# r9y9/deepvoice3_pytorch

Measured on NVIDIA H100. Metric: mel-frames/sec training step (B=16,T_mel=800), higher is better.
Workload: dtype f32 via split 16-bit pairs (fp16 pairs forward, bf16 pairs for gradients; 3 wgmma passes per product, fp32 accumulate)

## Files before the change

deepvoice3_pytorch_b200/csrc/tc_common.cuh:

```cuda
#pragma once
#include <cuda.h>
#include <cuda_bf16.h>
#include "common.cuh"

namespace dv3 {
namespace tc {

__device__ __forceinline__ uint32_t smem_u32(const void* p) { return (uint32_t)__cvta_generic_to_shared(p); }

__device__ __forceinline__ void mbar_init(uint64_t* bar, uint32_t count) {
    asm volatile("mbarrier.init.shared::cta.b64 [%0], %1;" ::"r"(smem_u32(bar)), "r"(count));
}
__device__ __forceinline__ void fence_barrier_init() {
    asm volatile("fence.mbarrier_init.release.cluster;" ::: "memory");
}
__device__ __forceinline__ void fence_proxy_async() {
    asm volatile("fence.proxy.async.shared::cta;" ::: "memory");
}
__device__ __forceinline__ void mbar_arrive_expect_tx(uint64_t* bar, uint32_t bytes) {
    asm volatile("mbarrier.arrive.expect_tx.shared::cta.b64 _, [%0], %1;" ::"r"(smem_u32(bar)), "r"(bytes)
                 : "memory");
}
__device__ __forceinline__ void mbar_arrive(uint64_t* bar) {
    asm volatile("mbarrier.arrive.shared::cta.b64 _, [%0];" ::"r"(smem_u32(bar)) : "memory");
}
__device__ __forceinline__ void mbar_wait(uint64_t* bar, uint32_t parity) {
    asm volatile(
        "{\n"
        ".reg .pred p;\n"
        "DV3_WAIT:\n"
        "mbarrier.try_wait.parity.shared::cta.b64 p, [%0], %1;\n"
        "@p bra DV3_DONE;\n"
        "bra DV3_WAIT;\n"
        "DV3_DONE:\n"
        "}\n" ::"r"(smem_u32(bar)),
        "r"(parity)
        : "memory");
}

__device__ __forceinline__ void tma_load_3d(void* smem_dst, const CUtensorMap* map, uint64_t* bar, int c0, int c1,
                                            int c2) {
    asm volatile(
        "cp.async.bulk.tensor.3d.shared::cluster.global.mbarrier::complete_tx::bytes [%0], [%1, {%3, %4, %5}], [%2];"
        ::"r"(smem_u32(smem_dst)), "l"(map), "r"(smem_u32(bar)), "r"(c0), "r"(c1), "r"(c2)
        : "memory");
}
__device__ __forceinline__ void prefetch_tmap(const CUtensorMap* map) {
    asm volatile("prefetch.tensormap [%0];" ::"l"(map) : "memory");
}
__device__ __forceinline__ void tma_store_3d(const CUtensorMap* map, const void* smem_src, int c0, int c1, int c2) {
    asm volatile("cp.async.bulk.tensor.3d.global.shared::cta.bulk_group [%0, {%2, %3, %4}], [%1];"
                 ::"l"(map), "r"(smem_u32(smem_src)), "r"(c0), "r"(c1), "r"(c2)
                 : "memory");
}
__device__ __forceinline__ void bulk_commit() { asm volatile("cp.async.bulk.commit_group;" ::: "memory"); }
__device__ __forceinline__ void bulk_wait_read() { asm volatile("cp.async.bulk.wait_group.read 0;" ::: "memory"); }
__device__ __forceinline__ void bulk_wait() { asm volatile("cp.async.bulk.wait_group 0;" ::: "memory"); }
__device__ __forceinline__ void mbar_arrive_cnt(uint64_t* bar, uint32_t count) {
    asm volatile("mbarrier.arrive.shared::cta.b64 _, [%0], %1;" ::"r"(smem_u32(bar)), "r"(count) : "memory");
}
__device__ __forceinline__ void named_bar_sync(int id, int threads) {
    asm volatile("bar.sync %0, %1;" ::"r"(id), "r"(threads) : "memory");
}

template <int N>
__device__ __forceinline__ void setmaxnreg_dec() { asm volatile("setmaxnreg.dec.sync.aligned.u32 %0;" ::"n"(N)); }
template <int N>
__device__ __forceinline__ void setmaxnreg_inc() { asm volatile("setmaxnreg.inc.sync.aligned.u32 %0;" ::"n"(N)); }

__device__ __forceinline__ void wgmma_fence() { asm volatile("wgmma.fence.sync.aligned;" ::: "memory"); }
__device__ __forceinline__ void wgmma_commit() { asm volatile("wgmma.commit_group.sync.aligned;" ::: "memory"); }
template <int N>
__device__ __forceinline__ void wgmma_wait() { asm volatile("wgmma.wait_group.sync.aligned %0;" ::"n"(N) : "memory"); }
__device__ __forceinline__ int frag_row(int i, int warp_in_wg, int lane) {
    return 16 * warp_in_wg + (lane >> 2) + 8 * ((i >> 1) & 1);
}
__device__ __forceinline__ int frag_col(int i, int lane) { return 8 * (i >> 2) + 2 * (lane & 3) + (i & 1); }

__device__ __forceinline__ uint64_t make_wgmma_desc(uint32_t saddr, uint32_t lbo, uint32_t sbo, uint32_t layout) {
    uint64_t d = 0;
    d |= (uint64_t)((saddr & 0x3FFFF) >> 4);
    d |= (uint64_t)((lbo >> 4) & 0x3FFF) << 16;
    d |= (uint64_t)((sbo >> 4) & 0x3FFF) << 32;
    d |= (uint64_t)layout << 62;
    return d;
}
constexpr uint32_t WG_SW128 = 1, WG_SW64 = 2;

template <int TA, int TB>
__device__ __forceinline__ void wgmma_f16_n64(float* d, uint64_t a, uint64_t b, uint32_t acc) {
    asm volatile(
        "{\n.reg .pred p;\nsetp.ne.b32 p, %34, 0;\n"
        "wgmma.mma_async.sync.aligned.m64n64k16.f32.f16.f16 {%0, %1, %2, %3, %4, %5, %6, %7, %8, %9, %10, %11, %12, %13, %14, %15, %16, %17, %18, %19, %20, %21, %22, %23, %24, %25, %26, %27, %28, %29, %30, %31}, %32, %33, p, 1, 1, %35, %36;\n}\n"
        : "+f"(d[0]), "+f"(d[1]), "+f"(d[2]), "+f"(d[3]), "+f"(d[4]), "+f"(d[5]), "+f"(d[6]), "+f"(d[7]), "+f"(d[8]), "+f"(d[9]), "+f"(d[10]), "+f"(d[11]), "+f"(d[12]), "+f"(d[13]), "+f"(d[14]), "+f"(d[15]), "+f"(d[16]), "+f"(d[17]), "+f"(d[18]), "+f"(d[19]), "+f"(d[20]), "+f"(d[21]), "+f"(d[22]), "+f"(d[23]), "+f"(d[24]), "+f"(d[25]), "+f"(d[26]), "+f"(d[27]), "+f"(d[28]), "+f"(d[29]), "+f"(d[30]), "+f"(d[31])
        : "l"(a), "l"(b), "r"(acc), "n"(TA), "n"(TB));
}
template <int TA, int TB>
__device__ __forceinline__ void wgmma_bf16_n64(float* d, uint64_t a, uint64_t b, uint32_t acc) {
    asm volatile(
        "{\n.reg .pred p;\nsetp.ne.b32 p, %34, 0;\n"
        "wgmma.mma_async.sync.aligned.m64n64k16.f32.bf16.bf16 {%0, %1, %2, %3, %4, %5, %6, %7, %8, %9, %10, %11, %12, %13, %14, %15, %16, %17, %18, %19, %20, %21, %22, %23, %24, %25, %26, %27, %28, %29, %30, %31}, %32, %33, p, 1, 1, %35, %36;\n}\n"
        : "+f"(d[0]), "+f"(d[1]), "+f"(d[2]), "+f"(d[3]), "+f"(d[4]), "+f"(d[5]), "+f"(d[6]), "+f"(d[7]), "+f"(d[8]), "+f"(d[9]), "+f"(d[10]), "+f"(d[11]), "+f"(d[12]), "+f"(d[13]), "+f"(d[14]), "+f"(d[15]), "+f"(d[16]), "+f"(d[17]), "+f"(d[18]), "+f"(d[19]), "+f"(d[20]), "+f"(d[21]), "+f"(d[22]), "+f"(d[23]), "+f"(d[24]), "+f"(d[25]), "+f"(d[26]), "+f"(d[27]), "+f"(d[28]), "+f"(d[29]), "+f"(d[30]), "+f"(d[31])
        : "l"(a), "l"(b), "r"(acc), "n"(TA), "n"(TB));
}
template <int TA, int TB>
__device__ __forceinline__ void wgmma_f16_n128(float* d, uint64_t a, uint64_t b, uint32_t acc) {
    asm volatile(
        "{\n.reg .pred p;\nsetp.ne.b32 p, %66, 0;\n"
        "wgmma.mma_async.sync.aligned.m64n128k16.f32.f16.f16 {%0, %1, %2, %3, %4, %5, %6, %7, %8, %9, %10, %11, %12, %13, %14, %15, %16, %17, %18, %19, %20, %21, %22, %23, %24, %25, %26, %27, %28, %29, %30, %31, %32, %33, %34, %35, %36, %37, %38, %39, %40, %41, %42, %43, %44, %45, %46, %47, %48, %49, %50, %51, %52, %53, %54, %55, %56, %57, %58, %59, %60, %61, %62, %63}, %64, %65, p, 1, 1, %67, %68;\n}\n"
        : "+f"(d[0]), "+f"(d[1]), "+f"(d[2]), "+f"(d[3]), "+f"(d[4]), "+f"(d[5]), "+f"(d[6]), "+f"(d[7]), "+f"(d[8]), "+f"(d[9]), "+f"(d[10]), "+f"(d[11]), "+f"(d[12]), "+f"(d[13]), "+f"(d[14]), "+f"(d[15]), "+f"(d[16]), "+f"(d[17]), "+f"(d[18]), "+f"(d[19]), "+f"(d[20]), "+f"(d[21]), "+f"(d[22]), "+f"(d[23]), "+f"(d[24]), "+f"(d[25]), "+f"(d[26]), "+f"(d[27]), "+f"(d[28]), "+f"(d[29]), "+f"(d[30]), "+f"(d[31]), "+f"(d[32]), "+f"(d[33]), "+f"(d[34]), "+f"(d[35]), "+f"(d[36]), "+f"(d[37]), "+f"(d[38]), "+f"(d[39]), "+f"(d[40]), "+f"(d[41]), "+f"(d[42]), "+f"(d[43]), "+f"(d[44]), "+f"(d[45]), "+f"(d[46]), "+f"(d[47]), "+f"(d[48]), "+f"(d[49]), "+f"(d[50]), "+f"(d[51]), "+f"(d[52]), "+f"(d[53]), "+f"(d[54]), "+f"(d[55]), "+f"(d[56]), "+f"(d[57]), "+f"(d[58]), "+f"(d[59]), "+f"(d[60]), "+f"(d[61]), "+f"(d[62]), "+f"(d[63])
        : "l"(a), "l"(b), "r"(acc), "n"(TA), "n"(TB));
}
template <int TA, int TB>
__device__ __forceinline__ void wgmma_bf16_n128(float* d, uint64_t a, uint64_t b, uint32_t acc) {
    asm volatile(
        "{\n.reg .pred p;\nsetp.ne.b32 p, %66, 0;\n"
        "wgmma.mma_async.sync.aligned.m64n128k16.f32.bf16.bf16 {%0, %1, %2, %3, %4, %5, %6, %7, %8, %9, %10, %11, %12, %13, %14, %15, %16, %17, %18, %19, %20, %21, %22, %23, %24, %25, %26, %27, %28, %29, %30, %31, %32, %33, %34, %35, %36, %37, %38, %39, %40, %41, %42, %43, %44, %45, %46, %47, %48, %49, %50, %51, %52, %53, %54, %55, %56, %57, %58, %59, %60, %61, %62, %63}, %64, %65, p, 1, 1, %67, %68;\n}\n"
        : "+f"(d[0]), "+f"(d[1]), "+f"(d[2]), "+f"(d[3]), "+f"(d[4]), "+f"(d[5]), "+f"(d[6]), "+f"(d[7]), "+f"(d[8]), "+f"(d[9]), "+f"(d[10]), "+f"(d[11]), "+f"(d[12]), "+f"(d[13]), "+f"(d[14]), "+f"(d[15]), "+f"(d[16]), "+f"(d[17]), "+f"(d[18]), "+f"(d[19]), "+f"(d[20]), "+f"(d[21]), "+f"(d[22]), "+f"(d[23]), "+f"(d[24]), "+f"(d[25]), "+f"(d[26]), "+f"(d[27]), "+f"(d[28]), "+f"(d[29]), "+f"(d[30]), "+f"(d[31]), "+f"(d[32]), "+f"(d[33]), "+f"(d[34]), "+f"(d[35]), "+f"(d[36]), "+f"(d[37]), "+f"(d[38]), "+f"(d[39]), "+f"(d[40]), "+f"(d[41]), "+f"(d[42]), "+f"(d[43]), "+f"(d[44]), "+f"(d[45]), "+f"(d[46]), "+f"(d[47]), "+f"(d[48]), "+f"(d[49]), "+f"(d[50]), "+f"(d[51]), "+f"(d[52]), "+f"(d[53]), "+f"(d[54]), "+f"(d[55]), "+f"(d[56]), "+f"(d[57]), "+f"(d[58]), "+f"(d[59]), "+f"(d[60]), "+f"(d[61]), "+f"(d[62]), "+f"(d[63])
        : "l"(a), "l"(b), "r"(acc), "n"(TA), "n"(TB));
}
template <int TA, int TB>
__device__ __forceinline__ void wgmma_f16_n256(float* d, uint64_t a, uint64_t b, uint32_t acc) {
    asm volatile(
        "{\n.reg .pred p;\nsetp.ne.b32 p, %130, 0;\n"
        "wgmma.mma_async.sync.aligned.m64n256k16.f32.f16.f16 {%0, %1, %2, %3, %4, %5, %6, %7, %8, %9, %10, %11, %12, %13, %14, %15, %16, %17, %18, %19, %20, %21, %22, %23, %24, %25, %26, %27, %28, %29, %30, %31, %32, %33, %34, %35, %36, %37, %38, %39, %40, %41, %42, %43, %44, %45, %46, %47, %48, %49, %50, %51, %52, %53, %54, %55, %56, %57, %58, %59, %60, %61, %62, %63, %64, %65, %66, %67, %68, %69, %70, %71, %72, %73, %74, %75, %76, %77, %78, %79, %80, %81, %82, %83, %84, %85, %86, %87, %88, %89, %90, %91, %92, %93, %94, %95, %96, %97, %98, %99, %100, %101, %102, %103, %104, %105, %106, %107, %108, %109, %110, %111, %112, %113, %114, %115, %116, %117, %118, %119, %120, %121, %122, %123, %124, %125, %126, %127}, %128, %129, p, 1, 1, %131, %132;\n}\n"
        : "+f"(d[0]), "+f"(d[1]), "+f"(d[2]), "+f"(d[3]), "+f"(d[4]), "+f"(d[5]), "+f"(d[6]), "+f"(d[7]), "+f"(d[8]), "+f"(d[9]), "+f"(d[10]), "+f"(d[11]), "+f"(d[12]), "+f"(d[13]), "+f"(d[14]), "+f"(d[15]), "+f"(d[16]), "+f"(d[17]), "+f"(d[18]), "+f"(d[19]), "+f"(d[20]), "+f"(d[21]), "+f"(d[22]), "+f"(d[23]), "+f"(d[24]), "+f"(d[25]), "+f"(d[26]), "+f"(d[27]), "+f"(d[28]), "+f"(d[29]), "+f"(d[30]), "+f"(d[31]), "+f"(d[32]), "+f"(d[33]), "+f"(d[34]), "+f"(d[35]), "+f"(d[36]), "+f"(d[37]), "+f"(d[38]), "+f"(d[39]), "+f"(d[40]), "+f"(d[41]), "+f"(d[42]), "+f"(d[43]), "+f"(d[44]), "+f"(d[45]), "+f"(d[46]), "+f"(d[47]), "+f"(d[48]), "+f"(d[49]), "+f"(d[50]), "+f"(d[51]), "+f"(d[52]), "+f"(d[53]), "+f"(d[54]), "+f"(d[55]), "+f"(d[56]), "+f"(d[57]), "+f"(d[58]), "+f"(d[59]), "+f"(d[60]), "+f"(d[61]), "+f"(d[62]), "+f"(d[63]), "+f"(d[64]), "+f"(d[65]), "+f"(d[66]), "+f"(d[67]), "+f"(d[68]), "+f"(d[69]), "+f"(d[70]), "+f"(d[71]), "+f"(d[72]), "+f"(d[73]), "+f"(d[74]), "+f"(d[75]), "+f"(d[76]), "+f"(d[77]), "+f"(d[78]), "+f"(d[79]), "+f"(d[80]), "+f"(d[81]), "+f"(d[82]), "+f"(d[83]), "+f"(d[84]), "+f"(d[85]), "+f"(d[86]), "+f"(d[87]), "+f"(d[88]), "+f"(d[89]), "+f"(d[90]), "+f"(d[91]), "+f"(d[92]), "+f"(d[93]), "+f"(d[94]), "+f"(d[95]), "+f"(d[96]), "+f"(d[97]), "+f"(d[98]), "+f"(d[99]), "+f"(d[100]), "+f"(d[101]), "+f"(d[102]), "+f"(d[103]), "+f"(d[104]), "+f"(d[105]), "+f"(d[106]), "+f"(d[107]), "+f"(d[108]), "+f"(d[109]), "+f"(d[110]), "+f"(d[111]), "+f"(d[112]), "+f"(d[113]), "+f"(d[114]), "+f"(d[115]), "+f"(d[116]), "+f"(d[117]), "+f"(d[118]), "+f"(d[119]), "+f"(d[120]), "+f"(d[121]), "+f"(d[122]), "+f"(d[123]), "+f"(d[124]), "+f"(d[125]), "+f"(d[126]), "+f"(d[127])
        : "l"(a), "l"(b), "r"(acc), "n"(TA), "n"(TB));
}
template <int TA, int TB>
__device__ __forceinline__ void wgmma_bf16_n256(float* d, uint64_t a, uint64_t b, uint32_t acc) {
    asm volatile(
        "{\n.reg .pred p;\nsetp.ne.b32 p, %130, 0;\n"
        "wgmma.mma_async.sync.aligned.m64n256k16.f32.bf16.bf16 {%0, %1, %2, %3, %4, %5, %6, %7, %8, %9, %10, %11, %12, %13, %14, %15, %16, %17, %18, %19, %20, %21, %22, %23, %24, %25, %26, %27, %28, %29, %30, %31, %32, %33, %34, %35, %36, %37, %38, %39, %40, %41, %42, %43, %44, %45, %46, %47, %48, %49, %50, %51, %52, %53, %54, %55, %56, %57, %58, %59, %60, %61, %62, %63, %64, %65, %66, %67, %68, %69, %70, %71, %72, %73, %74, %75, %76, %77, %78, %79, %80, %81, %82, %83, %84, %85, %86, %87, %88, %89, %90, %91, %92, %93, %94, %95, %96, %97, %98, %99, %100, %101, %102, %103, %104, %105, %106, %107, %108, %109, %110, %111, %112, %113, %114, %115, %116, %117, %118, %119, %120, %121, %122, %123, %124, %125, %126, %127}, %128, %129, p, 1, 1, %131, %132;\n}\n"
        : "+f"(d[0]), "+f"(d[1]), "+f"(d[2]), "+f"(d[3]), "+f"(d[4]), "+f"(d[5]), "+f"(d[6]), "+f"(d[7]), "+f"(d[8]), "+f"(d[9]), "+f"(d[10]), "+f"(d[11]), "+f"(d[12]), "+f"(d[13]), "+f"(d[14]), "+f"(d[15]), "+f"(d[16]), "+f"(d[17]), "+f"(d[18]), "+f"(d[19]), "+f"(d[20]), "+f"(d[21]), "+f"(d[22]), "+f"(d[23]), "+f"(d[24]), "+f"(d[25]), "+f"(d[26]), "+f"(d[27]), "+f"(d[28]), "+f"(d[29]), "+f"(d[30]), "+f"(d[31]), "+f"(d[32]), "+f"(d[33]), "+f"(d[34]), "+f"(d[35]), "+f"(d[36]), "+f"(d[37]), "+f"(d[38]), "+f"(d[39]), "+f"(d[40]), "+f"(d[41]), "+f"(d[42]), "+f"(d[43]), "+f"(d[44]), "+f"(d[45]), "+f"(d[46]), "+f"(d[47]), "+f"(d[48]), "+f"(d[49]), "+f"(d[50]), "+f"(d[51]), "+f"(d[52]), "+f"(d[53]), "+f"(d[54]), "+f"(d[55]), "+f"(d[56]), "+f"(d[57]), "+f"(d[58]), "+f"(d[59]), "+f"(d[60]), "+f"(d[61]), "+f"(d[62]), "+f"(d[63]), "+f"(d[64]), "+f"(d[65]), "+f"(d[66]), "+f"(d[67]), "+f"(d[68]), "+f"(d[69]), "+f"(d[70]), "+f"(d[71]), "+f"(d[72]), "+f"(d[73]), "+f"(d[74]), "+f"(d[75]), "+f"(d[76]), "+f"(d[77]), "+f"(d[78]), "+f"(d[79]), "+f"(d[80]), "+f"(d[81]), "+f"(d[82]), "+f"(d[83]), "+f"(d[84]), "+f"(d[85]), "+f"(d[86]), "+f"(d[87]), "+f"(d[88]), "+f"(d[89]), "+f"(d[90]), "+f"(d[91]), "+f"(d[92]), "+f"(d[93]), "+f"(d[94]), "+f"(d[95]), "+f"(d[96]), "+f"(d[97]), "+f"(d[98]), "+f"(d[99]), "+f"(d[100]), "+f"(d[101]), "+f"(d[102]), "+f"(d[103]), "+f"(d[104]), "+f"(d[105]), "+f"(d[106]), "+f"(d[107]), "+f"(d[108]), "+f"(d[109]), "+f"(d[110]), "+f"(d[111]), "+f"(d[112]), "+f"(d[113]), "+f"(d[114]), "+f"(d[115]), "+f"(d[116]), "+f"(d[117]), "+f"(d[118]), "+f"(d[119]), "+f"(d[120]), "+f"(d[121]), "+f"(d[122]), "+f"(d[123]), "+f"(d[124]), "+f"(d[125]), "+f"(d[126]), "+f"(d[127])
        : "l"(a), "l"(b), "r"(acc), "n"(TA), "n"(TB));
}

template <int N, int TA, int TB>
__device__ __forceinline__ void wgmma_mma(bool bf16, float* d, uint64_t a, uint64_t b, uint32_t acc) {
    if (N == 64) { if (bf16) wgmma_bf16_n64<TA, TB>(d, a, b, acc); else wgmma_f16_n64<TA, TB>(d, a, b, acc); }
    if (N == 128) { if (bf16) wgmma_bf16_n128<TA, TB>(d, a, b, acc); else wgmma_f16_n128<TA, TB>(d, a, b, acc); }
    if (N == 256) { if (bf16) wgmma_bf16_n256<TA, TB>(d, a, b, acc); else wgmma_f16_n256<TA, TB>(d, a, b, acc); }
}

}

int encode_tmap_bf16_3d(CUtensorMap* map, const void* base, uint64_t d0, uint64_t d1, uint64_t d2,
                        uint64_t stride1_bytes, uint64_t stride2_bytes, uint32_t box0, uint32_t box1);

}
```

deepvoice3_pytorch_b200/csrc/tc_gemm.cu:

```cuda
#include "tc_common.cuh"
#include "tc_ring.cuh"
#include "../../include/dv3b200.h"

namespace dv3 {

using namespace tc;

constexpr int TC_CONV_THREADS = 512;
constexpr int TC_PRODUCER_REGS = 24;
constexpr int TC_CONSUMER_REGS = 168;
constexpr int TC_EPILOGUE_REGS = 152;
static_assert(TC_PRODUCER_REGS <= 65536 / TC_CONV_THREADS && TC_CONSUMER_REGS >= 65536 / TC_CONV_THREADS &&
              TC_EPILOGUE_REGS >= 65536 / TC_CONV_THREADS, "setmaxnreg direction of each warpgroup");
static_assert(128 * TC_PRODUCER_REGS + 256 * TC_CONSUMER_REGS + 128 * TC_EPILOGUE_REGS <= 65536, "register file");
constexpr int MAX_TAPS_TC = 8;
enum { TC_GATED = 0, TC_CONV = 1 };

struct TcMaps { CUtensorMap a[2]; CUtensorMap b[2]; };

struct TcParams {
    int T;
    int Nc;
    int rows_per_tap;
    int k, kb_n;
    int tap_off[MAX_TAPS_TC];
    const float* bias; const float* spk; const float* res;
    float* y; float* save_a; float* save_s;
    int gate_mode, residual;
    float* out; const float* e1; const float* e2; float alpha; int addmode, relu;
    float p_drop; const unsigned long long* seed_ptr; uint32_t salt;
    float gmain;
    int operand_bf16;
    int tma_out;
};

template <int BK> struct SwizzleOf;
template <> struct SwizzleOf<64> { static constexpr uint32_t layout = WG_SW128, sbo = 1024; };
template <> struct SwizzleOf<32> { static constexpr uint32_t layout = WG_SW64, sbo = 512; };

template <int BK>
__device__ __forceinline__ uint64_t make_desc(uint32_t saddr) {
    return make_wgmma_desc(saddr, 16, SwizzleOf<BK>::sbo, SwizzleOf<BK>::layout);
}


template <int NC>
__device__ __forceinline__ int dense_at(int c) {
    const int r = threadIdx.x & 127;
    return (r >> 5) * NC * 32 + c * 32 + ((((r >> 2) & 7) ^ (c & 7)) << 2) + (r & 3);
}

struct TcOutMaps { CUtensorMap out[3]; CUtensorMap res; };

struct Handoff { float* tile; float* staging; uint64_t* acc_empty; uint64_t* in_full; };

__device__ __forceinline__ void release_tile(const Handoff& h, bool tma) {
    if (!tma) mbar_arrive(h.acc_empty);
    else if ((threadIdx.x & 127) == 0) {
        bulk_commit();
        bulk_wait_read();
        mbar_arrive_cnt(h.acc_empty, 128);
    }
}

template <int BR>
__device__ __forceinline__ void stage_residual(const TcParams& p, const TcOutMaps& om, const Handoff& h, int a_row0,
                                               int a_z, int b_row0) {
    if (!p.tma_out || !((p.gate_mode != 0) || p.residual) || (threadIdx.x & 127) != 0) return;
    mbar_arrive_expect_tx(h.in_full, 128 * BR * 4);
#pragma unroll
    for (int q = 0; q < 4; ++q) tma_load_3d(h.staging + q * BR * 32, &om.res, h.in_full, a_row0 + 32 * q, b_row0, a_z);
}

template <int BR>
__device__ __forceinline__ void epilogue_gated(const TcParams& p, const TcOutMaps& om, const Handoff& h, int n,
                                               int a_row0, int a_z, int b_row0) {
    constexpr int NC = 2 * BR;
    const int t = a_row0 + (threadIdx.x & 127), b = a_z, C = p.Nc;
    const bool tv = t < p.T, tma = p.tma_out != 0;
    const float* __restrict__ bias = p.bias;
    const float* __restrict__ res = p.res;
    const float* __restrict__ spk = p.spk;
    float* __restrict__ yo = p.y;
    float* __restrict__ ao = p.save_a;
    float* __restrict__ so = p.save_s;
    float* tile = h.tile;
    float* st = h.staging;
    const bool need_res = (p.gate_mode != 0) || p.residual;
    const size_t base = ((size_t)b * C + b_row0) * p.T + (tv ? t : 0);
    if (need_res) {
        if (tma) mbar_wait(h.in_full, n & 1);
        else {
#pragma unroll 8
            for (int c = 0; c < BR; ++c) st[dense_at<BR>(c)] = tv ? __ldg(&res[base + (size_t)c * p.T]) : 0.f;
        }
    }
#pragma unroll 1
    for (int c32 = 0; c32 < BR; c32 += 32) {
        float sp[32], ba[32], bb[32];
        const size_t cb = base + (size_t)c32 * p.T;
#pragma unroll
        for (int i = 0; i < 32; ++i) {
            ba[i] = __ldg(&bias[b_row0 + c32 + i]);
            bb[i] = __ldg(&bias[C + b_row0 + c32 + i]);
            if (spk) sp[i] = tv ? __ldg(&spk[cb + (size_t)i * p.T]) : 0.f;
        }
#pragma unroll
        for (int i = 0; i < 32; ++i) {
            const int cl = c32 + i;
            float va = tile[dense_at<NC>(cl)];
            if (spk) va += sp[i];
            const float a = va + ba[i];
            const float s = sigmoidf_(tile[dense_at<NC>(BR + cl)] + bb[i]);
            const float rr = need_res ? st[dense_at<BR>(cl)] : 0.f;
            float y;
            if (p.gate_mode == 0) {
                y = a * s;
                if (p.residual) y = (y + rr) * 0.70710678118654752f;
            } else {
                y = s * a + (1.f - s) * rr;
            }
            st[dense_at<BR>(cl)] = y;
            tile[dense_at<NC>(cl)] = a;
            tile[dense_at<NC>(BR + cl)] = s;
        }
    }
    if (tma) {
        fence_proxy_async();
        named_bar_sync(1, 128);
        if ((threadIdx.x & 127) == 0) {
#pragma unroll
            for (int q = 0; q < 4; ++q) {
                const int t0 = a_row0 + 32 * q;
                if (t0 >= p.T) break;
                tma_store_3d(&om.out[0], st + q * BR * 32, t0, b_row0, b);
                if (ao) tma_store_3d(&om.out[1], tile + q * NC * 32, t0, b_row0, b);
                if (so) tma_store_3d(&om.out[2], tile + q * NC * 32 + BR * 32, t0, b_row0, b);
            }
        }
    } else if (tv) {
#pragma unroll 8
        for (int c = 0; c < BR; ++c) {
            const size_t idx = base + (size_t)c * p.T;
            yo[idx] = st[dense_at<BR>(c)];
            if (ao) ao[idx] = tile[dense_at<NC>(c)];
            if (so) so[idx] = tile[dense_at<NC>(BR + c)];
        }
    }
    release_tile(h, tma);
}

template <int NCOLS>
__device__ __forceinline__ void epilogue_conv(const TcParams& p, const TcOutMaps& om, const Handoff& h, int a_row0,
                                              int a_z, int b_row0) {
    const int t = a_row0 + (threadIdx.x & 127), b = a_z;
    const bool tv = t < p.T, tma = p.tma_out != 0;
    const DropCfg drop = make_drop(p.p_drop, p.seed_ptr, p.salt);
    const float* __restrict__ bias = p.bias;
    const float* __restrict__ e1 = p.e1;
    const float* __restrict__ e2 = p.e2;
    float* __restrict__ out = p.out;
    float* tile = h.tile;
    const size_t base = ((size_t)b * p.Nc + b_row0) * p.T + (tv ? t : 0);
#pragma unroll 1
    for (int c32 = 0; c32 < NCOLS; c32 += 32) {
        float bz[32], v[32], x2[32];
        const int n0 = b_row0 + c32;
        const size_t cb = base + (size_t)c32 * p.T;
#pragma unroll
        for (int i = 0; i < 32; ++i) {
            const bool ok = tv && n0 + i < p.Nc;
            bz[i] = (bias && n0 + i < p.Nc) ? __ldg(&bias[n0 + i]) : 0.f;
            v[i] = (p.addmode != 0 && ok) ? __ldg(&e1[cb + (size_t)i * p.T]) : 0.f;
            x2[i] = (p.addmode == 2 && ok) ? __ldg(&e2[cb + (size_t)i * p.T]) : 0.f;
        }
#pragma unroll
        for (int i = 0; i < 32; ++i) {
            float& d = tile[dense_at<NCOLS>(c32 + i)];
            float g = d * drop_scale(drop, (uint32_t)(cb + (size_t)i * p.T));
            if (bias) g += bz[i];
            if (p.addmode == 1) g += p.alpha * v[i];
            else if (p.addmode == 2) g += v[i] * (1.f - x2[i]);
            if (p.relu) g = fmaxf(g, 0.f);
            d = g;
        }
    }
    if (tma) {
        fence_proxy_async();
        named_bar_sync(1, 128);
        if ((threadIdx.x & 127) == 0) {
#pragma unroll
            for (int q = 0; q < 4; ++q) {
                const int t0 = a_row0 + 32 * q;
                if (t0 >= p.T) break;
                tma_store_3d(&om.out[0], tile + q * NCOLS * 32, t0, b_row0, b);
            }
        }
    } else if (tv) {
#pragma unroll 8
        for (int c = 0; c < NCOLS; ++c)
            if (b_row0 + c < p.Nc) out[base + (size_t)c * p.T] = tile[dense_at<NCOLS>(c)];
    }
    release_tile(h, tma);
}

template <class Cfg, int NPL, class Decode, class Load, class Mma, class Gmain, class Epilogue, class Stage>
__device__ __forceinline__ void tc_pipeline(const TcMaps& maps, int num_units, Decode decode, Load load, Mma mma,
                                            Gmain gmain, Epilogue epilogue, Stage stage) {
    static_assert(NPL == 1 || NPL == 2, "one or two operand planes");
    static_assert(Cfg::NCOLS <= 128, "main + cross accumulators must fit in the registers of a consumer thread");
    static_assert(Cfg::STAGES >= 2, "pipeline needs at least two stages");
    constexpr int STAGE = Cfg::STAGE, STAGES = Cfg::STAGES;
    constexpr int NR = Cfg::NCOLS / 2;
    pdl_trigger();
    extern __shared__ uint8_t smem_raw[];
    uint8_t* smem = smem_raw + ((1024 - (smem_u32(smem_raw) & 1023)) & 1023);
    float* acc_tile = reinterpret_cast<float*>(smem + STAGES * STAGE);
    uint64_t* full = reinterpret_cast<uint64_t*>(smem + STAGES * STAGE + Cfg::ACC_TILE + Cfg::STAGING);
    uint64_t* empty = full + STAGES;
    uint64_t* acc_full = empty + STAGES;
    uint64_t* acc_empty = acc_full + 1;
    uint64_t* in_full = acc_empty + 1;
    const int warp = threadIdx.x >> 5, lane = threadIdx.x & 31;

    if (threadIdx.x == 0) {
#pragma unroll
        for (int pl = 0; pl < NPL; ++pl) prefetch_tmap(&maps.a[pl]);
#pragma unroll
        for (int pl = 0; pl < NPL; ++pl) prefetch_tmap(&maps.b[pl]);
        for (int s = 0; s < STAGES; ++s) { mbar_init(&full[s], 1); mbar_init(&empty[s], 2); }
        mbar_init(acc_full, 256);
        mbar_init(acc_empty, 128);
        mbar_init(in_full, 1);
        fence_barrier_init();
    }
    __syncthreads();
    pdl_wait();

    if (warp >= 12) {
        setmaxnreg_inc<TC_EPILOGUE_REGS>();
        const Handoff h = {acc_tile, acc_tile + Cfg::ACC_TILE / 4, acc_empty, in_full};
        if (blockIdx.x < num_units) stage(decode(blockIdx.x), h);
        int n = 0;
        for (int u = blockIdx.x; u < num_units; u += gridDim.x, ++n) {
            const auto w = decode(u);
            mbar_wait(acc_full, n & 1);
            epilogue(w, n, h);
            if (u + gridDim.x < num_units) stage(decode(u + gridDim.x), h);
        }
        if ((threadIdx.x & 127) == 0) bulk_wait();
    } else if (warp >= 8) {
        setmaxnreg_dec<TC_PRODUCER_REGS>();
        if (warp == 8 && lane == 0) {
            int it = 0;
            for (int u = blockIdx.x; u < num_units; u += gridDim.x) {
                const auto w = decode(u);
                for (int kit = 0; kit < w.n_iters; ++kit, ++it) {
                    const int s = it % STAGES, ph = (it / STAGES) & 1;
                    mbar_wait(&empty[s], ph ^ 1);
                    mbar_arrive_expect_tx(&full[s], STAGE);
                    load(w, kit, smem + s * STAGE, &full[s]);
                }
            }
        }
    } else {
        setmaxnreg_inc<TC_CONSUMER_REGS>();
        const int wg = warp >> 2, wq = warp & 3;
        float acc[NR], xacc[NPL == 2 ? NR : 1];
        int it = 0, n = 0;
        for (int u = blockIdx.x; u < num_units; u += gridDim.x, ++n) {
            const auto w = decode(u);
#pragma unroll
            for (int i = 0; i < NR; ++i) {
                acc[i] = 0.f;
                if constexpr (NPL == 2) xacc[i] = 0.f;
            }
            for (int kit = 0; kit < w.n_iters; ++kit, ++it) {
                const int s = it % STAGES, ph = (it / STAGES) & 1;
                mbar_wait(&full[s], ph);
                wgmma_fence();
                mma(smem + s * STAGE, wg, acc, xacc);
                wgmma_commit();
                wgmma_wait<1>();
                if (kit > 0 && (threadIdx.x & 127) == 0) mbar_arrive(&empty[(it - 1) % STAGES]);
            }
            wgmma_wait<0>();
            if (w.n_iters > 0 && (threadIdx.x & 127) == 0) mbar_arrive(&empty[(it - 1) % STAGES]);
            const float gm = gmain(w);
            mbar_wait(acc_empty, (n & 1) ^ 1);
            const int sw = (((wq & 1) << 2) | (lane >> 4)) ^ ((lane & 3) << 1);
            float* const frag0 = Cfg::DENSE ? acc_tile + (2 * wg + (wq >> 1)) * Cfg::NCOLS * 32 + (lane & 3) * 64 +
                                                  ((lane >> 2) & 3)
                                            : acc_tile;
#pragma unroll
            for (int i = 0; i < NR; ++i) {
                float* dst = Cfg::DENSE
                    ? frag0 + (i >> 2) * 256 + (i & 1) * 32 + ((sw ^ (i & 3)) << 2)
                    : &acc_tile[(64 * wg + frag_row(i, wq, lane)) * Cfg::ACC_PITCH + frag_col(i, lane)];
                if constexpr (NPL == 2) *dst = fmaf(xacc[i], LO_INV, acc[i] * gm);
                else *dst = acc[i] * gm;
            }
            mbar_arrive(acc_full);
        }
    }
}

template <int MODE, int NBOX, int BR, int BK, bool BF16, int NPL>
__global__ void __launch_bounds__(TC_CONV_THREADS, 1)
tc_conv_kernel(const __grid_constant__ TcMaps maps, const __grid_constant__ TcOutMaps om,
               const __grid_constant__ TcParams p, int tiles_x, int tiles_y, int num_tiles) {
    using Cfg = TcCfg<NBOX, BK, BR, NPL>;
    constexpr int NCOLS = Cfg::NCOLS;
    constexpr int TILE = 128 * BK * 2, TILE_B = BR * BK * 2;
    constexpr int B_OFF = NPL * TILE;
    constexpr int A_HALF = 64 * BK * 2;
    const int n_iters = p.k * p.kb_n;

    struct Tile { int a_row0, a_z, b_row0, b_row1, n_iters; };
    auto decode = [&](int tile) {
        Tile w;
        const int ty = tile % tiles_y, r = tile / tiles_y;
        w.a_z = r / tiles_x;
        w.a_row0 = (r % tiles_x) * 128;
        if (MODE == TC_GATED) { w.b_row0 = ty * BR; w.b_row1 = p.Nc + ty * BR; }
        else { w.b_row0 = ty * BR * NBOX; w.b_row1 = w.b_row0 + BR; }
        w.n_iters = n_iters;
        return w;
    };
    auto load = [&](const Tile& w, int kit, uint8_t* st, uint64_t* bar) {
        const int j = kit / p.kb_n, kb = kit - j * p.kb_n;
        const int ax = kb * BK, ay = w.a_row0 + p.tap_off[j];
        const int by0 = j * p.rows_per_tap + w.b_row0, by1 = j * p.rows_per_tap + w.b_row1;
#pragma unroll
        for (int pl = 0; pl < NPL; ++pl) {
            tma_load_3d(st + pl * TILE, &maps.a[pl], bar, ax, ay, w.a_z);
            uint8_t* bdst = st + B_OFF + pl * NBOX * TILE_B;
            tma_load_3d(bdst, &maps.b[pl], bar, ax, by0, 0);
            if (NBOX == 2) tma_load_3d(bdst + TILE_B, &maps.b[pl], bar, ax, by1, 0);
        }
    };
    auto mma = [&](const uint8_t* st, int wg, float* acc, float* xacc) {
        const uint32_t sa = smem_u32(st) + wg * A_HALF, sb = smem_u32(st + B_OFF);
#pragma unroll
        for (int kk = 0; kk < BK / 16; ++kk) {
            const uint32_t ko = kk * 32;
            const uint64_t a0 = make_desc<BK>(sa + ko), b0 = make_desc<BK>(sb + ko);
            wgmma_mma<NCOLS, 0, 0>(BF16, acc, a0, b0, 1);
            if constexpr (NPL == 2) {
                const uint64_t a1 = make_desc<BK>(sa + TILE + ko), b1 = make_desc<BK>(sb + NBOX * TILE_B + ko);
                wgmma_mma<NCOLS, 0, 0>(BF16, xacc, a0, b1, 1);
                wgmma_mma<NCOLS, 0, 0>(BF16, xacc, a1, b0, 1);
            }
        }
    };
    auto gmain = [&](const Tile&) { return p.gmain; };
    auto epilogue = [&](const Tile& w, int n, const Handoff& h) {
        if (MODE == TC_GATED) epilogue_gated<BR>(p, om, h, n, w.a_row0, w.a_z, w.b_row0);
        else epilogue_conv<NCOLS>(p, om, h, w.a_row0, w.a_z, w.b_row0);
    };
    auto stage = [&](const Tile& w, const Handoff& h) {
        if (MODE == TC_GATED) stage_residual<BR>(p, om, h, w.a_row0, w.a_z, w.b_row0);
    };
    tc_pipeline<Cfg, NPL>(maps, num_tiles, decode, load, mma, gmain, epilogue, stage);
}

struct TcMnParams {
    int T, B, Mw, Nw, k;
    int tap_off[MAX_TAPS_TC];
    int nsplit, batches_per_split, kb_n;
    int tiles_n, tiles_m, num_units;
    float* dw; long long split_stride;
    int msplit; long long s_m, s_mh, s_n, s_j;
    float gcoef;
};

template <int NPL>
__global__ void __launch_bounds__(TC_CONV_THREADS, 1)
tc_wgrad_mn_kernel(const __grid_constant__ TcMaps maps, const __grid_constant__ TcMnParams p) {
    using Cfg = WgCfg<NPL>;
    constexpr int A_PL = 2 * WG_BOX, B_PL = 2 * WG_BOX;
    constexpr uint32_t LBO = 4096, SBO = 1024;

    struct Unit { int m0, n0, j, s, b_beg, n_iters; };
    auto decode = [&](int u) {
        Unit w;
        w.n0 = (u % p.tiles_n) * 128;
        int r = u / p.tiles_n;
        w.m0 = (r % p.tiles_m) * 128;
        r /= p.tiles_m;
        w.j = r % p.k;
        w.s = r / p.k;
        w.b_beg = w.s * p.batches_per_split;
        const int b_end = min(p.B, w.b_beg + p.batches_per_split);
        w.n_iters = (b_end > w.b_beg ? b_end - w.b_beg : 0) * p.kb_n;
        return w;
    };
    auto load = [&](const Unit& w, int kit, uint8_t* st, uint64_t* bar) {
        const int bi = kit / p.kb_n, tc_ = kit - bi * p.kb_n;
        const int b = w.b_beg + bi, t0 = tc_ * 32;
#pragma unroll
        for (int pl = 0; pl < NPL; ++pl) {
#pragma unroll
            for (int h = 0; h < 2; ++h)
                tma_load_3d(st + pl * A_PL + h * WG_BOX, &maps.a[pl], bar, w.m0 + h * 64, t0, b);
#pragma unroll
            for (int q = 0; q < 2; ++q)
                tma_load_3d(st + NPL * A_PL + pl * B_PL + q * WG_BOX, &maps.b[pl], bar, w.n0 + q * 64,
                            t0 + p.tap_off[w.j], b);
        }
    };
    auto mma = [&](const uint8_t* st, int wg, float* acc, float* xacc) {
        const uint32_t sa = smem_u32(st);
#pragma unroll
        for (int kk = 0; kk < 2; ++kk) {
            const uint32_t ko = kk * 16 * 128;
            const uint64_t a0 = make_wgmma_desc(sa + wg * WG_BOX + ko, LBO, SBO, WG_SW128);
            const uint64_t b0 = make_wgmma_desc(sa + NPL * A_PL + ko, LBO, SBO, WG_SW128);
            wgmma_mma<128, 1, 1>(true, acc, a0, b0, 1);
            if constexpr (NPL == 2) {
                const uint64_t a1 = make_wgmma_desc(sa + A_PL + wg * WG_BOX + ko, LBO, SBO, WG_SW128);
                const uint64_t b1 = make_wgmma_desc(sa + 2 * A_PL + B_PL + ko, LBO, SBO, WG_SW128);
                wgmma_mma<128, 1, 1>(true, xacc, a0, b1, 1);
                wgmma_mma<128, 1, 1>(true, xacc, a1, b0, 1);
            }
        }
    };
    auto gmain = [&](const Unit& w) { return 1.f + p.gcoef * (float)(2 * w.n_iters); };
    auto epilogue = [&](const Unit& w, int, const Handoff& h) {
        const float* acc_tile = h.tile;
        const int r = threadIdx.x & 127;
        float* __restrict__ out = p.dw + (size_t)w.s * p.split_stride + (size_t)w.j * p.s_j;
        const int rows = min(128, p.Mw - w.m0), cols = min(128, p.Nw - w.n0);
        if (p.s_n == 1) {
            if (r < cols) {
                float* __restrict__ o = out + w.n0 + r;
#pragma unroll 4
                for (int i = 0; i < rows; ++i) {
                    const int m = w.m0 + i;
                    o[(size_t)(m % p.msplit) * p.s_m + (size_t)(m / p.msplit) * p.s_mh] = acc_tile[i * Cfg::ACC_PITCH + r];
                }
            }
        } else if (r < rows) {
            const int m = w.m0 + r;
            float* __restrict__ o = out + (size_t)(m % p.msplit) * p.s_m + (size_t)(m / p.msplit) * p.s_mh +
                                    (size_t)w.n0 * p.s_n;
            const float* arow = acc_tile + r * Cfg::ACC_PITCH;
#pragma unroll 4
            for (int c = 0; c < cols; ++c) o[(size_t)c * p.s_n] = arow[c];
        }
        mbar_arrive(h.acc_empty);
    };
    tc_pipeline<Cfg, NPL>(maps, p.num_units, decode, load, mma, gmain, epilogue, [](const Unit&, const Handoff&) {});
}

typedef CUresult (*EncodeTiledFn)(CUtensorMap*, CUtensorMapDataType, cuuint32_t, void*, const cuuint64_t*,
                                  const cuuint64_t*, const cuuint32_t*, const cuuint32_t*, CUtensorMapInterleave,
                                  CUtensorMapSwizzle, CUtensorMapL2promotion, CUtensorMapFloatOOBfill);

static EncodeTiledFn encode_fn() {
    static const EncodeTiledFn fn = [] {
        void* f = nullptr;
        cudaDriverEntryPointQueryResult qres;
        cudaError_t e = cudaGetDriverEntryPoint("cuTensorMapEncodeTiled", &f, cudaEnableDefault, &qres);
        return (e == cudaSuccess) ? (EncodeTiledFn)f : (EncodeTiledFn) nullptr;
    }();
    return fn;
}

int encode_tmap_bf16_3d(CUtensorMap* map, const void* base, uint64_t d0, uint64_t d1, uint64_t d2,
                        uint64_t stride1_bytes, uint64_t stride2_bytes, uint32_t box0, uint32_t box1) {
    const EncodeTiledFn enc = encode_fn();
    if (!enc) { set_error("cuTensorMapEncodeTiled entry point unavailable"); return 1; }
    cuuint64_t dims[3] = {d0, d1, d2};
    cuuint64_t strides[2] = {stride1_bytes, stride2_bytes};
    cuuint32_t box[3] = {box0, box1, 1};
    cuuint32_t estr[3] = {1, 1, 1};
    const CUtensorMapSwizzle sw = box0 * 2 == 128 ? CU_TENSOR_MAP_SWIZZLE_128B : CU_TENSOR_MAP_SWIZZLE_64B;
    CUresult r = enc(map, CU_TENSOR_MAP_DATA_TYPE_BFLOAT16, 3, const_cast<void*>(base), dims, strides, box, estr,
                     CU_TENSOR_MAP_INTERLEAVE_NONE, sw, CU_TENSOR_MAP_L2_PROMOTION_L2_256B,
                     CU_TENSOR_MAP_FLOAT_OOB_FILL_NONE);
    if (r != CUDA_SUCCESS) {
        set_error("cuTensorMapEncodeTiled failed (%d): dims=(%llu,%llu,%llu) strides=(%llu,%llu) box=(%u,%u)", (int)r,
                  (unsigned long long)d0, (unsigned long long)d1, (unsigned long long)d2,
                  (unsigned long long)stride1_bytes, (unsigned long long)stride2_bytes, box0, box1);
        return 1;
    }
    return 0;
}

static int encode_tmap_f32_bct(CUtensorMap* map, const float* base, int B, int Nc, int T, int box_c) {
    const EncodeTiledFn enc = encode_fn();
    if (!enc) { set_error("cuTensorMapEncodeTiled entry point unavailable"); return 1; }
    cuuint64_t dims[3] = {(cuuint64_t)T, (cuuint64_t)Nc, (cuuint64_t)B};
    cuuint64_t strides[2] = {(cuuint64_t)T * 4, (cuuint64_t)Nc * T * 4};
    cuuint32_t box[3] = {32, (cuuint32_t)box_c, 1};
    cuuint32_t estr[3] = {1, 1, 1};
    CUresult r = enc(map, CU_TENSOR_MAP_DATA_TYPE_FLOAT32, 3, const_cast<float*>(base), dims, strides, box, estr,
                     CU_TENSOR_MAP_INTERLEAVE_NONE, CU_TENSOR_MAP_SWIZZLE_128B, CU_TENSOR_MAP_L2_PROMOTION_L2_256B,
                     CU_TENSOR_MAP_FLOAT_OOB_FILL_NONE);
    if (r != CUDA_SUCCESS) {
        set_error("cuTensorMapEncodeTiled failed (%d): fp32 (B,C,T) = (%d,%d,%d) box=(32,%d)", (int)r, B, Nc, T, box_c);
        return 1;
    }
    return 0;
}

static bool tma_rows(const float* base, int T) { return T % 4 == 0 && ((uintptr_t)base & 15) == 0; }

template <typename K>
static int ensure_smem(K kern, int bytes, const char* what) {
    cudaError_t e = cudaFuncSetAttribute(kern, cudaFuncAttributeMaxDynamicSharedMemorySize, bytes);
    if (e != cudaSuccess) { set_error("%s: cannot set %d B dynamic smem: %s", what, bytes, cudaGetErrorString(e)); return 1; }
    return 0;
}

template <class Cfg, auto kern, typename... Args>
static int launch_persistent(int units, cudaStream_t st, const char* what, const Args&... args) {
    static const int configured = ensure_smem(kern, Cfg::SMEM, what);
    if (configured) return 1;
    const int sms = config().sms, grid = units < sms ? units : sms;
    cudaError_t e = launch_k(kern, dim3(grid), dim3(TC_CONV_THREADS), (size_t)Cfg::SMEM, st, args...);
    if (e != cudaSuccess) { set_error("%s: launch failed: %s", what, cudaGetErrorString(e)); return 1; }
    return check_launch(what);
}

template <int MODE, int NBOX, int BR, int BK, bool BF16, int NPL>
static int launch_conv_fmt(const TcMaps& maps, const TcOutMaps& om, const TcParams& p, int tiles_x, int tiles_y,
                           int batch, cudaStream_t st, const char* what) {
    const int num_tiles = tiles_x * tiles_y * batch;
    return launch_persistent<TcCfg<NBOX, BK, BR, NPL>, tc_conv_kernel<MODE, NBOX, BR, BK, BF16, NPL>>(
        num_tiles, st, what, maps, om, p, tiles_x, tiles_y, num_tiles);
}

template <int MODE, int NBOX, int BR, int BK, int NPL = 2>
static int launch_conv(const TcMaps& maps, const TcOutMaps& om, const TcParams& p, int tiles_x, int tiles_y, int batch,
                       cudaStream_t st, const char* what) {
    if (p.operand_bf16)
        return launch_conv_fmt<MODE, NBOX, BR, BK, true, NPL>(maps, om, p, tiles_x, tiles_y, batch, st, what);
    return launch_conv_fmt<MODE, NBOX, BR, BK, false, NPL>(maps, om, p, tiles_x, tiles_y, batch, st, what);
}

static void fill_taps_tc(int* tap_off, int k, int dilation, int causal, bool transpose) {
    const int padl = causal ? (k - 1) * dilation : (k - 1) / 2 * dilation;
    for (int j = 0; j < MAX_TAPS_TC; ++j)
        tap_off[j] = j < k ? (transpose ? (padl - j * dilation) : (j * dilation - padl)) : 0;
}

static inline const void* plane(const void* base, int pl, long long plane_elems) {
    return (const char*)base + (size_t)pl * plane_elems * 2;
}

}

using namespace dv3;

extern "C" {

int dv3_tc_supported(int B, int C, int T, int k) {
    return (C % 128 == 0) && T >= 1 && k >= 1 && k <= MAX_TAPS_TC && B >= 1 && B <= 65535;
}
int dv3_tc_conv_supported(int B, int Cin, int Cout, int T, int k) {
    return T >= 1 && k >= 1 && k <= MAX_TAPS_TC && B >= 1 && B <= 65535 && (k == 1 || Cout % 128 == 0) && Cin >= 8 &&
           Cout >= 1;
}

int dv3_tc_convblock_fwd(const void* xd, const void* w, int npl, const float* bias, const float* spk,
                         const float* res, float* y, float* save_a, float* save_s, int B, int C, int T, int k,
                         int dilation, int causal, int mode, int residual, const void* fuse, void* stream) {
    DV3_REQUIRE(dv3_tc_supported(B, C, T, k), "tc_convblock_fwd: unsupported shape B=%d C=%d T=%d k=%d", B, C, T, k);
    DV3_REQUIRE(npl == 1 || npl == 2, "tc_convblock_fwd: npl must be 1 or 2");
    DV3_REQUIRE(fuse == nullptr, "tc_convblock_fwd: fuse must be NULL");
    TcMaps maps;
    const int t_tiles = (T + 127) / 128;
    const int BK = npl == 2 ? 32 : 64;
    for (int pl = 0; pl < npl; ++pl) {
        if (encode_tmap_bf16_3d(&maps.a[pl], plane(xd, pl, (long long)B * T * C), C, T, B, (uint64_t)C * 2,
                                (uint64_t)T * C * 2, BK, 128)) return 1;
        if (encode_tmap_bf16_3d(&maps.b[pl], plane(w, pl, (long long)k * 2 * C * C), C, (uint64_t)k * 2 * C, 1,
                                (uint64_t)C * 2, (uint64_t)k * 2 * C * C * 2, BK, 64)) return 1;
    }
    TcParams p = {};
    p.T = T; p.Nc = C; p.rows_per_tap = 2 * C; p.k = k; p.kb_n = C / BK;
    fill_taps_tc(p.tap_off, k, dilation, causal, false);
    p.bias = bias; p.spk = spk; p.res = res; p.y = y; p.save_a = save_a; p.save_s = save_s;
    p.gate_mode = mode; p.residual = residual;
    p.gmain = 1.f + config().tc_gamma * (float)(p.k * p.kb_n * (BK / 16));
    const bool need_res = mode != 0 || residual;
    TcOutMaps om = {};
    p.tma_out = tma_rows(y, T) && (!save_a || tma_rows(save_a, T)) && (!save_s || tma_rows(save_s, T)) &&
                (!need_res || tma_rows(res, T));
    if (p.tma_out) {
        const float* outs[3] = {y, save_a, save_s};
        for (int i = 0; i < 3; ++i)
            if (outs[i] && encode_tmap_f32_bct(&om.out[i], outs[i], B, C, T, 64)) return 1;
        if (need_res && encode_tmap_f32_bct(&om.res, res, B, C, T, 64)) return 1;
    }
    cudaStream_t st = (cudaStream_t)stream;
    if (npl == 1)
        return launch_conv_fmt<TC_GATED, 2, 64, 64, false, 1>(maps, om, p, t_tiles, C / 64, B, st, "tc_convblock_fwd");
    return launch_conv_fmt<TC_GATED, 2, 64, 32, false, 2>(maps, om, p, t_tiles, C / 64, B, st, "tc_convblock_fwd");
}

int dv3_tc_conv(const void* a, const void* w, int npl, float* out, int B, int Kc, int Nc, int T, int k, int dilation,
// ... 113 lines not shown
```

Measured before the change: 1.693 million.

## Split last-tile epilogue across consumer warpgroups and prefetch epilogue inputs to L2

For each CTA's final tile, the two consumer warpgroups, now idle, join the epilogue warpgroup and each handles an interleaved share of channel chunks, with the TMA store issued by one lead thread after a widened named barrier. For non-final tiles the epilogue issues L2 prefetches of the next tile's speaker, e1 and e2 inputs while staging the residual. The wgrad epilogue also replaces per-row div/mod with incremental counters. This targets the serialized epilogue tail at the end of the persistent loop, at the cost of extra barrier coordination and more register pressure in the consumer warpgroups.

```diff
diff --git a/deepvoice3_pytorch_b200/csrc/tc_common.cuh b/deepvoice3_pytorch_b200/csrc/tc_common.cuh
--- a/deepvoice3_pytorch_b200/csrc/tc_common.cuh
+++ b/deepvoice3_pytorch_b200/csrc/tc_common.cuh
@@ -47,6 +47,9 @@
 }
 __device__ __forceinline__ void prefetch_tmap(const CUtensorMap* map) {
     asm volatile("prefetch.tensormap [%0];" ::"l"(map) : "memory");
+}
+__device__ __forceinline__ void prefetch_l2(const void* p) {
+    asm volatile("prefetch.global.L2 [%0];" ::"l"(p));
 }
 __device__ __forceinline__ void tma_store_3d(const CUtensorMap* map, const void* smem_src, int c0, int c1, int c2) {
     asm volatile("cp.async.bulk.tensor.3d.global.shared::cta.bulk_group [%0, {%2, %3, %4}], [%1];"
diff --git a/deepvoice3_pytorch_b200/csrc/tc_gemm.cu b/deepvoice3_pytorch_b200/csrc/tc_gemm.cu
--- a/deepvoice3_pytorch_b200/csrc/tc_gemm.cu
+++ b/deepvoice3_pytorch_b200/csrc/tc_gemm.cu
@@ -13,6 +13,8 @@
 static_assert(TC_PRODUCER_REGS <= 65536 / TC_CONV_THREADS && TC_CONSUMER_REGS >= 65536 / TC_CONV_THREADS &&
               TC_EPILOGUE_REGS >= 65536 / TC_CONV_THREADS, "setmaxnreg direction of each warpgroup");
 static_assert(128 * TC_PRODUCER_REGS + 256 * TC_CONSUMER_REGS + 128 * TC_EPILOGUE_REGS <= 65536, "register file");
+constexpr int TC_EPILOGUE_LEAD = 3 * 128;
+constexpr int TC_LAST_PARTS = 3;
 constexpr int MAX_TAPS_TC = 8;
 enum { TC_GATED = 0, TC_CONV = 1 };
 
@@ -55,11 +57,23 @@
 struct Handoff { float* tile; float* staging; uint64_t* acc_empty; uint64_t* in_full; };
 
 __device__ __forceinline__ void release_tile(const Handoff& h, bool tma) {
+    if (threadIdx.x < TC_EPILOGUE_LEAD) return;
     if (!tma) mbar_arrive(h.acc_empty);
-    else if ((threadIdx.x & 127) == 0) {
+    else if (threadIdx.x == TC_EPILOGUE_LEAD) {
         bulk_commit();
         bulk_wait_read();
         mbar_arrive_cnt(h.acc_empty, 128);
+    }
+}
+
+__device__ __forceinline__ void prefetch_bct(const float* x, int T, int C, int b, int c0, int nc, int t0) {
+    const int ta = t0 + 32 * ((threadIdx.x >> 5) & 3), lane = threadIdx.x & 31;
+    if (ta >= T) return;
+    const int tb = min(ta + 31, T - 1);
+    for (int c = lane; c < nc && c0 + c < C; c += 32) {
+        const float* row = x + ((size_t)b * C + c0 + c) * T;
+        prefetch_l2(row + ta);
+        prefetch_l2(row + tb);
     }
 }
 
@@ -72,10 +86,11 @@
     for (int q = 0; q < 4; ++q) tma_load_3d(h.staging + q * BR * 32, &om.res, h.in_full, a_row0 + 32 * q, b_row0, a_z);
 }
 
-template <int BR>
+template <int BR, int CW>
 __device__ __forceinline__ void epilogue_gated(const TcParams& p, const TcOutMaps& om, const Handoff& h, int n,
-                                               int a_row0, int a_z, int b_row0) {
+                                               int a_row0, int a_z, int b_row0, int part, int nparts) {
     constexpr int NC = 2 * BR;
+    static_assert(BR % CW == 0, "whole channel chunks");
     const int t = a_row0 + (threadIdx.x & 127), b = a_z, C = p.Nc;
     const bool tv = t < p.T, tma = p.tma_out != 0;
     const float* __restrict__ bias = p.bias;
@@ -88,25 +103,23 @@
     float* st = h.staging;
     const bool need_res = (p.gate_mode != 0) || p.residual;
     const size_t base = ((size_t)b * C + b_row0) * p.T + (tv ? t : 0);
-    if (need_res) {
-        if (tma) mbar_wait(h.in_full, n & 1);
-        else {
+    if (need_res && tma) mbar_wait(h.in_full, n & 1);
+#pragma unroll 1
+    for (int c32 = part * CW; c32 < BR; c32 += nparts * CW) {
+        float sp[CW], ba[CW], bb[CW];
+        const size_t cb = base + (size_t)c32 * p.T;
+        if (need_res && !tma) {
 #pragma unroll 8
-            for (int c = 0; c < BR; ++c) st[dense_at<BR>(c)] = tv ? __ldg(&res[base + (size_t)c * p.T]) : 0.f;
-        }
-    }
-#pragma unroll 1
-    for (int c32 = 0; c32 < BR; c32 += 32) {
-        float sp[32], ba[32], bb[32];
-        const size_t cb = base + (size_t)c32 * p.T;
-#pragma unroll
-        for (int i = 0; i < 32; ++i) {
+            for (int i = 0; i < CW; ++i) st[dense_at<BR>(c32 + i)] = tv ? __ldg(&res[cb + (size_t)i * p.T]) : 0.f;
+        }
+#pragma unroll
+        for (int i = 0; i < CW; ++i) {
             ba[i] = __ldg(&bias[b_row0 + c32 + i]);
             bb[i] = __ldg(&bias[C + b_row0 + c32 + i]);
             if (spk) sp[i] = tv ? __ldg(&spk[cb + (size_t)i * p.T]) : 0.f;
         }
 #pragma unroll
-        for (int i = 0; i < 32; ++i) {
+        for (int i = 0; i < CW; ++i) {
             const int cl = c32 + i;
             float va = tile[dense_at<NC>(cl)];
             if (spk) va += sp[i];
@@ -127,8 +140,8 @@
     }
     if (tma) {
         fence_proxy_async();
-        named_bar_sync(1, 128);
-        if ((threadIdx.x & 127) == 0) {
+        named_bar_sync(1, 128 * nparts);
+        if (threadIdx.x == TC_EPILOGUE_LEAD) {
 #pragma unroll
             for (int q = 0; q < 4; ++q) {
                 const int t0 = a_row0 + 32 * q;
@@ -139,20 +152,24 @@
             }
         }
     } else if (tv) {
+#pragma unroll 1
+        for (int c32 = part * CW; c32 < BR; c32 += nparts * CW) {
 #pragma unroll 8
-        for (int c = 0; c < BR; ++c) {
-            const size_t idx = base + (size_t)c * p.T;
-            yo[idx] = st[dense_at<BR>(c)];
-            if (ao) ao[idx] = tile[dense_at<NC>(c)];
-            if (so) so[idx] = tile[dense_at<NC>(BR + c)];
+            for (int c = c32; c < c32 + CW; ++c) {
+                const size_t idx = base + (size_t)c * p.T;
+                yo[idx] = st[dense_at<BR>(c)];
+                if (ao) ao[idx] = tile[dense_at<NC>(c)];
+                if (so) so[idx] = tile[dense_at<NC>(BR + c)];
+            }
         }
     }
     release_tile(h, tma);
 }
 
-template <int NCOLS>
+template <int NCOLS, int CW>
 __device__ __forceinline__ void epilogue_conv(const TcParams& p, const TcOutMaps& om, const Handoff& h, int a_row0,
-                                              int a_z, int b_row0) {
+                                              int a_z, int b_row0, int part, int nparts) {
+    static_assert(NCOLS % CW == 0, "whole channel chunks");
     const int t = a_row0 + (threadIdx.x & 127), b = a_z;
     const bool tv = t < p.T, tma = p.tma_out != 0;
     const DropCfg drop = make_drop(p.p_drop, p.seed_ptr, p.salt);
@@ -163,19 +180,19 @@
     float* tile = h.tile;
     const size_t base = ((size_t)b * p.Nc + b_row0) * p.T + (tv ? t : 0);
 #pragma unroll 1
-    for (int c32 = 0; c32 < NCOLS; c32 += 32) {
-        float bz[32], v[32], x2[32];
+    for (int c32 = part * CW; c32 < NCOLS; c32 += nparts * CW) {
+        float bz[CW], v[CW], x2[CW];
         const int n0 = b_row0 + c32;
         const size_t cb = base + (size_t)c32 * p.T;
 #pragma unroll
-        for (int i = 0; i < 32; ++i) {
+        for (int i = 0; i < CW; ++i) {
             const bool ok = tv && n0 + i < p.Nc;
             bz[i] = (bias && n0 + i < p.Nc) ? __ldg(&bias[n0 + i]) : 0.f;
             v[i] = (p.addmode != 0 && ok) ? __ldg(&e1[cb + (size_t)i * p.T]) : 0.f;
             x2[i] = (p.addmode == 2 && ok) ? __ldg(&e2[cb + (size_t)i * p.T]) : 0.f;
         }
 #pragma unroll
-        for (int i = 0; i < 32; ++i) {
+        for (int i = 0; i < CW; ++i) {
             float& d = tile[dense_at<NCOLS>(c32 + i)];
             float g = d * drop_scale(drop, (uint32_t)(cb + (size_t)i * p.T));
             if (bias) g += bz[i];
@@ -187,8 +204,8 @@
     }
     if (tma) {
         fence_proxy_async();
-        named_bar_sync(1, 128);
-        if ((threadIdx.x & 127) == 0) {
+        named_bar_sync(1, 128 * nparts);
+        if (threadIdx.x == TC_EPILOGUE_LEAD) {
 #pragma unroll
             for (int q = 0; q < 4; ++q) {
                 const int t0 = a_row0 + 32 * q;
@@ -197,9 +214,12 @@
             }
         }
     } else if (tv) {
+#pragma unroll 1
+        for (int c32 = part * CW; c32 < NCOLS; c32 += nparts * CW) {
 #pragma unroll 8
-        for (int c = 0; c < NCOLS; ++c)
-            if (b_row0 + c < p.Nc) out[base + (size_t)c * p.T] = tile[dense_at<NCOLS>(c)];
+            for (int c = c32; c < c32 + CW; ++c)
+                if (b_row0 + c < p.Nc) out[base + (size_t)c * p.T] = tile[dense_at<NCOLS>(c)];
+        }
     }
     release_tile(h, tma);
 }
@@ -244,11 +264,14 @@
         int n = 0;
         for (int u = blockIdx.x; u < num_units; u += gridDim.x, ++n) {
             const auto w = decode(u);
+            const bool last = u + gridDim.x >= num_units;
             mbar_wait(acc_full, n & 1);
-            epilogue(w, n, h);
-            if (u + gridDim.x < num_units) stage(decode(u + gridDim.x), h);
-        }
-        if ((threadIdx.x & 127) == 0) bulk_wait();
+            if (last) epilogue(w, n, h, TC_LAST_PARTS - 1, TC_LAST_PARTS);
+            else {
+                epilogue(w, n, h, 0, 1);
+                stage(decode(u + gridDim.x), h);
+            }
+        }
     } else if (warp >= 8) {
         setmaxnreg_dec<TC_PRODUCER_REGS>();
         if (warp == 8 && lane == 0) {
@@ -301,6 +324,11 @@
                 else *dst = acc[i] * gm;
             }
             mbar_arrive(acc_full);
+            if (u + gridDim.x >= num_units) {
+                const Handoff h = {acc_tile, acc_tile + Cfg::ACC_TILE / 4, acc_empty, in_full};
+                mbar_wait(acc_full, n & 1);
+                epilogue(w, n, h, wg, TC_LAST_PARTS);
+            }
         }
     }
 }
@@ -354,12 +382,23 @@
         }
     };
     auto gmain = [&](const Tile&) { return p.gmain; };
-    auto epilogue = [&](const Tile& w, int n, const Handoff& h) {
-        if (MODE == TC_GATED) epilogue_gated<BR>(p, om, h, n, w.a_row0, w.a_z, w.b_row0);
-        else epilogue_conv<NCOLS>(p, om, h, w.a_row0, w.a_z, w.b_row0);
+    auto epilogue = [&](const Tile& w, int n, const Handoff& h, int part, int nparts) {
+        if (MODE == TC_GATED) {
+            if (nparts == 1) epilogue_gated<BR, 32>(p, om, h, n, w.a_row0, w.a_z, w.b_row0, 0, 1);
+            else epilogue_gated<BR, BR / 8>(p, om, h, n, w.a_row0, w.a_z, w.b_row0, part, nparts);
+        } else {
+            if (nparts == 1) epilogue_conv<NCOLS, 32>(p, om, h, w.a_row0, w.a_z, w.b_row0, 0, 1);
+            else epilogue_conv<NCOLS, NCOLS / 8>(p, om, h, w.a_row0, w.a_z, w.b_row0, part, nparts);
+        }
     };
     auto stage = [&](const Tile& w, const Handoff& h) {
-        if (MODE == TC_GATED) stage_residual<BR>(p, om, h, w.a_row0, w.a_z, w.b_row0);
+        if (MODE == TC_GATED) {
+            stage_residual<BR>(p, om, h, w.a_row0, w.a_z, w.b_row0);
+            if (p.spk) prefetch_bct(p.spk, p.T, p.Nc, w.a_z, w.b_row0, BR, w.a_row0);
+        } else {
+            if (p.addmode != 0) prefetch_bct(p.e1, p.T, p.Nc, w.a_z, w.b_row0, NCOLS, w.a_row0);
+            if (p.addmode == 2) prefetch_bct(p.e2, p.T, p.Nc, w.a_z, w.b_row0, NCOLS, w.a_row0);
+        }
     };
     tc_pipeline<Cfg, NPL>(maps, num_tiles, decode, load, mma, gmain, epilogue, stage);
 }
@@ -426,18 +465,24 @@
         }
     };
     auto gmain = [&](const Unit& w) { return 1.f + p.gcoef * (float)(2 * w.n_iters); };
-    auto epilogue = [&](const Unit& w, int, const Handoff& h) {
+    auto epilogue = [&](const Unit& w, int, const Handoff& h, int part, int nparts) {
         const float* acc_tile = h.tile;
         const int r = threadIdx.x & 127;
+        const int cw = nparts == 1 ? 128 : 16;
         float* __restrict__ out = p.dw + (size_t)w.s * p.split_stride + (size_t)w.j * p.s_j;
         const int rows = min(128, p.Mw - w.m0), cols = min(128, p.Nw - w.n0);
         if (p.s_n == 1) {
             if (r < cols) {
                 float* __restrict__ o = out + w.n0 + r;
+#pragma unroll 1
+                for (int i0 = part * cw; i0 < rows; i0 += nparts * cw) {
+                    const int i1 = min(i0 + cw, rows);
+                    int mr = (w.m0 + i0) % p.msplit, mq = (w.m0 + i0) / p.msplit;
 #pragma unroll 4
-                for (int i = 0; i < rows; ++i) {
-                    const int m = w.m0 + i;
-                    o[(size_t)(m % p.msplit) * p.s_m + (size_t)(m / p.msplit) * p.s_mh] = acc_tile[i * Cfg::ACC_PITCH + r];
+                    for (int i = i0; i < i1; ++i) {
+                        o[(size_t)mr * p.s_m + (size_t)mq * p.s_mh] = acc_tile[i * Cfg::ACC_PITCH + r];
+                        if (++mr == p.msplit) { mr = 0; ++mq; }
+                    }
                 }
             }
         } else if (r < rows) {
@@ -445,10 +490,14 @@
             float* __restrict__ o = out + (size_t)(m % p.msplit) * p.s_m + (size_t)(m / p.msplit) * p.s_mh +
                                     (size_t)w.n0 * p.s_n;
             const float* arow = acc_tile + r * Cfg::ACC_PITCH;
+#pragma unroll 1
+            for (int c0 = part * cw; c0 < cols; c0 += nparts * cw) {
+                const int c1 = min(c0 + cw, cols);
 #pragma unroll 4
-            for (int c = 0; c < cols; ++c) o[(size_t)c * p.s_n] = arow[c];
-        }
-        mbar_arrive(h.acc_empty);
+                for (int c = c0; c < c1; ++c) o[(size_t)c * p.s_n] = arow[c];
+            }
+        }
+        if (threadIdx.x >= TC_EPILOGUE_LEAD) mbar_arrive(h.acc_empty);
     };
     tc_pipeline<Cfg, NPL>(maps, p.num_units, decode, load, mma, gmain, epilogue, [](const Unit&, const Handoff&) {});
 }
```

New measurement: 1.749 million, median of 6. +3.3%, better.
